# h-walk/PySlice

Measured on AMD Instinct MI355X. Metric: slice-steps/sec (probes x frames x slices / s), potential + slice loop + exit FFT, higher is better.
Workload: dtype complex64 (f32); 1 GPU; 64-probe STEM grid, 1024x1024 grid, 200 slices, 54 MD frames per GPU (BASELINE configs[2] per-frame work), 106583 atoms, 30 mrad, 100 keV; grid=1024, slices=200, probes=64, parallelism=frames x1, world_size_checked=1, frame_slots=59, frame_batch=4

## Files before the change

pyslice_amd/build_native.py:

```python
from __future__ import annotations

import os
import shutil
import subprocess
import sys

HERE = os.path.dirname(os.path.abspath(__file__))
CSRC = os.path.join(HERE, "csrc")
OUT = os.path.join(HERE, "libmslice.so")
SOURCES = ["mslice.hip", "slice_pass.hip", "slice_mixed_a.hip", "slice_mixed_b.hip", "slice_mixed_c.hip", "slice_mixed_d.hip", "slice_mixed_e.hip", "slice_mixed_f.hip", "tacaw_direct.hip", "tacaw_split.hip", "tacaw_split2.hip", "tacaw_welch.hip"]
def _deps():
    return sorted(f for f in os.listdir(CSRC) if f.endswith((".hip", ".h"))) + [os.path.join("..", "..", "include", "mslice.h")]
ARCH = "gfx950"


def _hipcc():
    for cand in (os.environ.get("HIPCC"), shutil.which("hipcc"), "/opt/rocm/bin/hipcc"):
        if cand and os.path.exists(cand):
            return cand
    raise RuntimeError("hipcc not found (ROCm toolchain required to build libmslice.so)")


def needs_build() -> bool:
    if not os.path.exists(OUT):
        return True
    t = os.path.getmtime(OUT)
    for d in _deps():
        p = os.path.join(CSRC, d)
        if os.path.exists(p) and os.path.getmtime(p) > t:
            return True
    return False


def build(force: bool = False, verbose: bool = True) -> str:
    if not force and not needs_build():
        return OUT
    from concurrent.futures import ThreadPoolExecutor
    objdir = os.path.join(HERE, "build")
    os.makedirs(objdir, exist_ok=True)
    flags = [f"--offload-arch={ARCH}", "-O3", "-std=c++17", "-fno-slp-vectorize", "-fPIC"]

    def compile_one(src):
        obj = os.path.join(objdir, os.path.splitext(src)[0] + ".o")
        cmd = [_hipcc()] + flags + ["-c", "-o", obj, src]
        if verbose:
            print("[pyslice_amd] " + " ".join(cmd), flush=True)
        subprocess.run(cmd, cwd=CSRC, check=True)
        return obj

    with ThreadPoolExecutor(max_workers=min(len(SOURCES), os.cpu_count() or 1)) as pool:
        objs = list(pool.map(compile_one, SOURCES))
    cmd = [_hipcc(), f"--offload-arch={ARCH}", "-shared", "-fPIC", "-o", OUT] + objs
    if verbose:
        print("[pyslice_amd] " + " ".join(cmd), flush=True)
    subprocess.run(cmd, cwd=CSRC, check=True)
    return OUT


if __name__ == "__main__":
    build(force="--force" in sys.argv)
    print(OUT)
```

pyslice_amd/csrc/mslice.hip:

```cpp
#include <hip/hip_runtime.h>

#include <algorithm>
#include <cmath>
#include <cstdarg>
#include <cstdio>
#include <cstdlib>
#include <cstring>
#include <string>
#include <type_traits>
#include <vector>

#include "../../include/mslice.h"
#include "fft_generic.h"
#include "fft_pow2.h"
#include "pot_ifft.h"
#include "rowtm_pass.h"
#include "potential.h"
#include "absorptive.h"
#include "finite.h"
#include "tds.h"
#include "ionization.h"
#include "slice_sums.h"
#include "thermal.h"
#include "phonons.h"
// ... 968 lines not shown
    case AX_TWO:
        job.tw = o.tw; job.tw2 = o.tw2; job.pl = o.ptab;
        return paired_dispatch(job, [&](auto in_p, auto out_p) { return launch_rowT2_io<decltype(in_p)::value, decltype(out_p)::value>(h, job, kind); });
    case AX_FOURSTEP:
        job.tw = (&o == &h->opx) ? h->tw4_x : h->tw4_y;
        return o.R == 32 ? launch_rowT_r<32>(h, job, kind) : launch_rowT_r<16>(h, job, kind);
    default:
        return fail(h, MSL_ERR_STATE, "transposing pass: the axis has no one-pass kernel");
    }
}

int slice_loop_onepass_b(msl_handle* h, int fused_slot, int groups, int first_group) {
    const msl_config& c = h->cfg;
    const int P = c.n_probes * groups, nz = c.nz;
    const size_t toff = (size_t)first_group * c.nz * c.nx * c.ny;
    const size_t npix = (size_t)c.nx * c.ny;
    const long long isA = (long long)c.nx * h->pitch, isB = (long long)c.ny * h->pitchT;
    const bool fused = fused_slot >= 0;
    int rc;
    if ((rc = begin_timed(h, nz + 4 + (fused ? tap_launches(h) : 0)))) return rc;
    for (int k = 0; k < nz; ++k) {
        RowTJob j{};
        j.flags = (k > 0 ? P2_PRE_A : 0) | (k < nz - 1 ? P2_POST_A : 0);
        if (h->debug_flags_mask >= 0) j.flags &= h->debug_flags_mask;
        j.n_images = P;
        set_frame_groups(h, j, groups);
        if (h->opx.kind == AX_WAVE2K && h->opy.kind == AX_WAVE2K)
            j.flags |= (k > 0 ? P2_IN_PAIRED : 0) | (k < nz - 1 ? P2_OUT_PAIRED : 0);
        if (interleaves(h->opx) && interleaves(h->opy) && !dbg_env("MSL_NO_INTERLEAVE") && h->debug_flags_mask < 0) {
            j.flags |= (k > 0 ? P2_IN_PAIRED : 0) | (k < nz - 1 ? P2_OUT_PAIRED : 0);
            j.perm_shift = (((k & 1) ? h->opy : h->opx).R == 32) ? 2 : 1;
        }
        if (!(k & 1)) {
            j.in = (k == 0) ? h->psi0 : h->psi; j.out = h->psiT;
            j.trans = h->trans + toff + (size_t)k * npix; j.pl = h->pyt;
            j.in_image_stride = isA; j.out_image_stride = isB; j.in_pitch = h->pitch; j.out_pitch = h->pitchT; j.n_lines = c.nx;
            rc = launch_rowT_dir(h, h->opy, j, K_ROW);
        } else {
            j.in = h->psiT; j.out = h->psi;
            j.trans = h->transT + toff + (size_t)k * npix; j.pl = h->pxt;
            j.in_image_stride = isB; j.out_image_stride = isA; j.in_pitch = h->pitchT; j.out_pitch = h->pitch; j.n_lines = c.ny;
            rc = launch_rowT_dir(h, h->opx, j, K_COL);
        }
        if (rc) return rc;
        if (k < nz - 1) {
            int rp = 0;
            const int order = tap_order((k & 1) ? h->opx : h->opy, j.flags, j.perm_shift, &rp);
            if ((rc = tap_step(h, k, fused_slot, groups, (k & 1) ? h->psi : h->psiT, !(k & 1), order, rp, (k & 1) ? 1 : 0))) return rc;
        }
    }
    if (nz & 1) {
        dim3 grid((c.nx + 31) / 32, (c.ny + 31) / 32, P);
        hipLaunchKernelGGL(transpose_kernel, grid, dim3(256), 0, h->stream, h->psiT, h->psi, c.ny, c.nx, h->pitchT, h->pitch, isB, isA);
        HIPCHK(h, hipGetLastError());
        if ((rc = mark_launch(h, K_OTHER))) return rc;
    }
    if (fused) {
        if (h->Ry) {
            RowJob r = row_job(h, h->psi, P, h->pitch);
            r.do_fft = true;
            if ((rc = launch_row_fast(h, r, K_OTHER))) return rc;
        } else {
            LineArgs r = row_args(h, h->psi, h->psi, P, h->pitch);
            r.fft1 = +1;
            if ((rc = launch_lines(h, h->plan_y, r, K_OTHER))) return rc;
        }
        if ((rc = epilogue_x_pass(h, fused_slot, groups))) return rc;
    }
    count_slice_loop(h, P, groups, fused, 16);
    return MSL_OK;
}

template <int R>
int launch_row2_r(msl_handle* h, Row2Job job, int kind) {
    constexpr int N = R * R, G = 256 / R;
    const size_t lds = (size_t)N * 16 + (size_t)G * R * (R + 1) * 4;
    const int per_cu = std::max(1, std::min(2, (int)((size_t)h->lds_limit / lds)));
    const int grid = chunked_grid(h, job, job.nx / G, (long long)h->n_cus * per_cu);
    hipLaunchKernelGGL(row_pass2_kernel<R>, dim3(grid), dim3(256), lds, h->stream, job);
    HIPCHK(h, hipGetLastError());
    return mark_launch(h, kind);
}

int slice_loop_onepass(msl_handle* h, int fused_slot, int groups, int first_group) {
    if (h->scheme_b) return slice_loop_onepass_b(h, fused_slot, groups, first_group);
    const msl_config& c = h->cfg;
    const int P = c.n_probes * groups, nz = c.nz;
    const size_t toff = (size_t)first_group * c.nz * c.nx * c.ny;
    const size_t npix = (size_t)c.nx * c.ny;
    const long long isA = (long long)c.nx * h->pitch, isB = (long long)c.ny * h->pitchT;
    const bool fused = fused_slot >= 0;
    int rc;
    if (nz == 1)
        HIPCHK(h, hipMemcpyAsync(h->psi, h->psi0, (size_t)P * isA * sizeof(float2), hipMemcpyDeviceToDevice, h->stream));
    if ((rc = begin_timed(h, nz + 2 + (fused ? tap_launches(h) : 0)))) return rc;
    for (int k = 0; k < nz; ++k) {
        const bool last = (k == nz - 1);
        int flags = (k > 0 ? P2_PRE_A : 0) | (!last ? P2_POST_A : 0) | ((last && fused) ? P2_POST_F : 0);
        if (h->debug_flags_mask >= 0) flags &= h->debug_flags_mask;
        if (last) {
            Row2Job j{};
            j.psi = h->psi; j.trans = h->trans + toff + (size_t)k * npix; j.py = h->pyt; j.tw = h->tw4_y;
            j.image_stride = isA; j.pitch = h->pitch; j.nx = c.nx; j.n_images = P; j.flags = flags;
            set_frame_groups(h, j, groups);
            rc = h->Ry == 32 ? launch_row2_r<32>(h, j, K_ROW) : launch_row2_r<16>(h, j, K_ROW);
            if (rc) return rc;
            break;
        }
        const bool along_y = !slice_is_transposed(h, k);
        RowTJob j{};
        if (!dbg_env("MSL_NO_INTERLEAVE") && h->debug_flags_mask < 0) flags |= (k > 0 ? P2_IN_PAIRED : 0) | (k < nz - 2 ? P2_OUT_PAIRED : 0);
        j.flags = flags; j.n_images = P;
        j.perm_shift = ((along_y ? h->Rx : h->Ry) == 32) ? 2 : 1;
        set_frame_groups(h, j, groups);
        if (along_y) {
            j.in = (k == 0) ? h->psi0 : h->psi; j.out = h->psiT;
            j.trans = h->trans + toff + (size_t)k * npix; j.pl = h->pyt; j.tw = h->tw4_y;
            j.in_image_stride = isA; j.out_image_stride = isB; j.in_pitch = h->pitch; j.out_pitch = h->pitchT; j.n_lines = c.nx;
            rc = h->Ry == 32 ? launch_rowT_r<32>(h, j, K_ROW) : launch_rowT_r<16>(h, j, K_ROW);
        } else {
            j.in = (k == 0) ? h->psi0T : h->psiT; j.out = h->psi;
            j.trans = h->transT + toff + (size_t)k * npix; j.pl = h->pxt; j.tw = h->tw4_x;
            j.in_image_stride = isB; j.out_image_stride = isA; j.in_pitch = h->pitchT; j.out_pitch = h->pitch; j.n_lines = c.ny;
            rc = h->Rx == 32 ? launch_rowT_r<32>(h, j, K_COL) : launch_rowT_r<16>(h, j, K_COL);
        }
        if (rc) return rc;
        const int order = (j.flags & P2_OUT_PAIRED) ? TAP_INTERLEAVED : TAP_NATURAL;
        if ((rc = tap_step(h, k, fused_slot, groups, along_y ? h->psiT : h->psi, along_y, order, 8 << j.perm_shift, along_y ? 0 : 1))) return rc;
    }
    if (fused && (rc = epilogue_x_pass(h, fused_slot, groups))) return rc;
    count_slice_loop(h, P, groups, fused, 16);
    return MSL_OK;
}

int ensure_atoms(msl_handle* h, size_t n, size_t rows) {
    int rc;
    if (rows <= h->atom_cap) return (h->fin_R > 0 && h->d_wgt.n < h->atom_cap) ? h->d_wgt.alloc(h, h->atom_cap) : MSL_OK;
    (void)n;
    size_t cap = std::max<size_t>(rows, h->atom_cap * 3 / 2 + 1024);
    if (h->fin_R > 0 && (rc = h->d_wgt.alloc(h, cap))) return rc;
    if ((rc = h->d_pos.alloc(h, cap * 3)) || (rc = h->d_Z.alloc(h, cap)) || (rc = h->d_key.alloc(h, cap)) || (rc = h->d_order.alloc(h, cap)) ||
        (rc = h->d_u1.alloc(h, cap)) || (rc = h->d_u2.alloc(h, cap))) return rc;
    if ((rc = h->d_ex.alloc(h, cap * (size_t)(h->cfg.nx / 2 + 1))) || (rc = h->d_ey.alloc(h, cap * (size_t)(h->cfg.ny / 2 + 1)))) return rc;
    h->atom_cap = cap;
    return MSL_OK;
}

struct TdsSignal : TdsSums {
    static constexpr const char* name = "tds";
    static constexpr const char* setter = "msl_set_tds";
    static int slots(int n) { return n; }
    static int slab_slots(int n) { return n; }
    template <typename F> static void with_slots(int k, F&& f) { with_int<1, 2, 3, 4>(k, f); }
    static bool on(const msl_handle* h) { return h->tds_on; }
    static bool built(const msl_handle* h) { return h->tds_W && h->abs_built; }
    static int n(const msl_handle* h) { return h->tds_n; }
    static const float* weights(const msl_handle* h) { return h->tds_W; }
    static DevBuf<double>& slab(msl_handle* h) { return h->tds_part; }
};
struct IonSignal : IonSums {
    static constexpr const char* name = "ionization";
    static constexpr const char* setter = "msl_set_ionization";
    static int slots(int n) { return n <= 1 ? 1 : n <= 2 ? 2 : n <= 4 ? 4 : 8; }
    static int slab_slots(int) { return ION_MAX; }
    template <typename F> static void with_slots(int k, F&& f) { with_int<1, 2, 4, 8>(k, f); }
    static bool on(const msl_handle* h) { return h->ion_on; }
    static bool built(const msl_handle* h) { return h->ion_W && h->ion_built; }
    static int n(const msl_handle* h) { return h->ion_n; }
    static const float* weights(const msl_handle* h) { return h->ion_W; }
    static DevBuf<float>& slab(msl_handle* h) { return h->ion_part; }
};

template <class S>
int slice_sums_queue(msl_handle* h, const float2* psi, int P, const float* w, size_t w_cs, int n, double* dst, int reps = 1) {
    const msl_config& c = h->cfg;
    const long long pairs = (long long)c.nx * ((c.ny + 1) / 2), n_tiles = (pairs + S::TILE - 1) / S::TILE;
    if (n_tiles > 0x7fffffffLL) return fail(h, MSL_ERR_UNSUPPORTED, "%s: too many tiles", S::name);
    const int slots = S::slots(n);
    auto& part = S::slab(h);
    int rc = part.reserve(h, (size_t)n_tiles * P * S::slab_slots(n));
    if (rc) return rc;
    const long long wg_slots = (long long)h->n_cus * 8;
    int pc = P;
    while (pc > 1 && n_tiles * ((P + pc - 1) / pc) < wg_slots) pc = (pc + 1) / 2;
    while ((P + pc - 1) / pc > 65535) ++pc;
    const bool vec = (h->pitch % 2 == 0) && (((uintptr_t)psi & 15) == 0);
    const dim3 grid((unsigned)n_tiles, (unsigned)((P + pc - 1) / pc));
    for (int r = 0; r < reps; ++r) {
        S::with_slots(slots, [&](auto k) { with_bool(vec, [&](auto v) {
            hipLaunchKernelGGL((slice_sums_kernel<typename S::kernel_policy, decltype(k)::value, decltype(v)::value>), grid, dim3(256), 0, h->stream,
                               psi, w, (long long)w_cs, n, c.nx, c.ny, h->pitch, P, pc, part.p);
        }); });
        HIPCHK(h, hipGetLastError());
        if (reps == 1 && (rc = mark_launch(h, K_OTHER))) return rc;
    }
    S::with_slots(slots, [&](auto k) {
        hipLaunchKernelGGL((slice_sums_finish_kernel<typename S::acc_t, decltype(k)::value>), dim3((unsigned)(((long long)P * slots + 255) / 256)),
                           dim3(256), 0, h->stream, part.p, n_tiles, P, n, dst);
    });
    HIPCHK(h, hipGetLastError());
    return reps == 1 ? mark_launch(h, K_OTHER) : MSL_OK;
}

template <class S>
int slice_sums_of_slice(msl_handle* h, const float2* psi, int P, int z, double* dst, int reps = 1) {
    const size_t npix = (size_t)h->cfg.nx * h->cfg.ny;
    return slice_sums_queue<S>(h, psi, P, S::weights(h) + (size_t)z * npix, npix * h->cfg.nz, S::n(h), dst, reps);
}
int slice_sums_hook(msl_handle* h, int P, int z) {
    return h->tds_on ? slice_sums_of_slice<TdsSignal>(h, h->psi, P, z, h->tds_acc + (size_t)z * P * h->tds_n)
                     : slice_sums_of_slice<IonSignal>(h, h->psi, P, z, h->ion_acc + (size_t)z * P * h->ion_n);
}

// ... 3506 lines not shown
```

pyslice_amd/csrc/rowt_pass.h:

```cpp
#pragma once
#include <type_traits>
#include <utility>
#include <hip/hip_runtime.h>
#include "fft_regs.h"
#include "kernel_util.h"
#include "rowt_frame.h"

#ifndef MSL_TW_LDS
#define MSL_TW_LDS 0
#endif
#ifndef MSL_DIT_LCH
#define MSL_DIT_LCH 8
#endif
#ifndef MSL_DIT_FENCE
#define MSL_DIT_FENCE 0
#endif
#ifndef MSL_STAGGER
#define MSL_STAGGER 4
#endif
#define MSL_IC(x) std::integral_constant<int, (x)>{}

namespace msl {


template <int R>
__device__ __forceinline__ void exchange_addtid(float2 (&v)[R], const float* scratch_base, unsigned wave_scratch, int ln, int lane64) {
    static_assert(64 % R == 0 && R % 4 == 0, "R-lane groups inside one wave; rows are read four floats at a time");
    constexpr int PW = 68;
    if constexpr (MSL_ABL2 & 4) return;
    const float* rd = scratch_base + ln * PW + (lane64 / R) * R;
    asm volatile("s_mov_b32 m0, %0\n\ts_nop 1" :: "s"(wave_scratch) : "memory");
#pragma unroll
    for (int k1 = 0; k1 < R; ++k1) asm volatile("ds_write_addtid_b32 %0 offset:%1" :: "v"(v[k1].x), "n"(k1 * PW * 4) : "memory");
    wave_lds_fence();
#pragma unroll
    for (int g = 0; g < R / 4; ++g) {
        const float4 q = *reinterpret_cast<const float4*>(rd + 4 * g);
        v[4 * g].x = q.x; v[4 * g + 1].x = q.y; v[4 * g + 2].x = q.z; v[4 * g + 3].x = q.w;
    }
    wave_lds_fence();
    asm volatile("s_mov_b32 m0, %0\n\ts_nop 1" :: "s"(wave_scratch) : "memory");
#pragma unroll
    for (int k1 = 0; k1 < R; ++k1) asm volatile("ds_write_addtid_b32 %0 offset:%1" :: "v"(v[k1].y), "n"(k1 * PW * 4) : "memory");
    wave_lds_fence();
#pragma unroll
    for (int g = 0; g < R / 4; ++g) {
        const float4 q = *reinterpret_cast<const float4*>(rd + 4 * g);
        v[4 * g].y = q.x; v[4 * g + 1].y = q.y; v[4 * g + 2].y = q.z; v[4 * g + 3].y = q.w;
    }
    wave_lds_fence();
}

template <int R, bool INV, int WMODE, int STRIDE, int C0, typename TabPtr, int... J>
__device__ __forceinline__ void dit_leaf_chunk(const float2* in, float2* v, TabPtr tab, int ln, std::integer_sequence<int, J...>) {
    constexpr int LR = dit_leaf_radix(R), C = R / LR;
    float2 w[sizeof...(J)][4];
    if constexpr (MSL_ABL2 & 16) {
        ((w[J][0] = tab[ln], w[J][1] = tab[ln], w[J][2] = tab[ln], w[J][3] = tab[ln]), ...);
    } else {
        ((w[J][0] = tab[(C0 + J) * STRIDE + ln], w[J][1] = tab[(C0 + J + C) * STRIDE + ln]), ...);
        if constexpr (LR == 4) ((w[J][2] = tab[(C0 + J + 2 * C) * STRIDE + ln], w[J][3] = tab[(C0 + J + 3 * C) * STRIDE + ln]), ...);
    }
    (dit_leaf<R, INV, WMODE, C0 + J>(in, v, w[J]), ...);
    (pin(v[C0 + J]), ...); (pin(v[C0 + J + C]), ...);
    if constexpr (LR == 4) { (pin(v[C0 + J + 2 * C]), ...); (pin(v[C0 + J + 3 * C]), ...); }
    __builtin_amdgcn_sched_barrier(0);
}
template <int R, bool INV, int WMODE, int STRIDE, int CH, int C0, typename TabPtr>
__device__ __forceinline__ void dit_leaf_chunks(const float2* in, float2* v, TabPtr tab, int ln) {
    if constexpr (C0 < dit_leaf_count(R)) {
        dit_leaf_chunk<R, INV, WMODE, STRIDE, C0>(in, v, tab, ln, std::make_integer_sequence<int, CH>{});
        dit_leaf_chunks<R, INV, WMODE, STRIDE, CH, C0 + CH>(in, v, tab, ln);
    }
}

template <int R, bool INV, int WMODE, int K, int I>
__device__ __forceinline__ void dit_leaves_regs_part(const float2* in, float2* v, const float2* w) {
    if constexpr (I < K) {
        constexpr int LR = dit_leaf_radix(R);
        float2 ww[4];
        ww[0] = w[I]; ww[1] = w[I + K];
        if constexpr (LR == 4) { ww[2] = w[I + 2 * K]; ww[3] = w[I + 3 * K]; }
        dit_leaf<R, INV, WMODE, I>(in, v, ww);
        dit_leaves_regs_part<R, INV, WMODE, K, I + 1>(in, v, w);
    }
}
constexpr int rowT_tw_reg_leaves(int R, int FL) { return (!MSL_TW_LDS && R == 32 && FL >= 0) ? 8 : 0; }
constexpr int ROWT_TW_REG_LCH = 4;

constexpr int rowT_cs(int R) { return (R * R + 33) / 32 * 32 + 2; }
template <int R, int LINES, bool IN_P, bool OUT_P, int FL>
__global__ void __launch_bounds__(LINES * R, (R == 16) ? 3 : 2) rowT_pass_kernel(RowTJob job) {
    constexpr int N = R * R;
    constexpr int NT = LINES * R;
    constexpr int CS = rowT_cs(R);
    constexpr int TWK = rowT_tw_reg_leaves(R, FL), LRW = dit_leaf_radix(R);
    constexpr bool TWR = TWK > 0;
    constexpr int LCH0 = TWR ? ROWT_TW_REG_LCH : MSL_DIT_LCH;
    constexpr int LCHL = LCH0 < dit_leaf_count(R) ? LCH0 : dit_leaf_count(R);
    constexpr int FN = MSL_DIT_FENCE;
    static_assert(LINES == 16, "16 lines = 128-byte transposed segments (8 lines / 64 bytes measured 1.6x slower)");
    static_assert(dit_leaf_count(R) % LCHL == 0 && TWK % LCHL == 0 && TWK < dit_leaf_count(R), "whole chunks");
    extern __shared__ __attribute__((aligned(16))) char smem_raw[];
    float2* tw = reinterpret_cast<float2*>(smem_raw);
    float2* pl = tw + N;
    float2* tile = pl + N;
    const int tid = threadIdx.x;
    for (int i = tid; i < N; i += NT) { tw[i] = job.tw[i]; pl[i] = job.pl[i]; }
    __syncthreads();
    const int grp = tid / R, ln = tid % R;
    float2 twr[TWR ? LRW * TWK : 1];
    if constexpr (TWR) {
#pragma unroll
        for (int i = 0; i < LRW * TWK; ++i) twr[i] = tw[((i % TWK) + (i / TWK) * dit_leaf_count(R)) * R + ln];
        pin_all(twr);
    }
    const int l64 = tid & 63;
    float2* myrow = tile + grp * CS;
    const float* wscr = reinterpret_cast<const float*>(tile + (grp - grp % (64 / R)) * CS);
    const unsigned wscr_lds = __builtin_amdgcn_readfirstlane((unsigned)(size_t)(tile + (grp - grp % (64 / R)) * CS));
    const bool pre_a = (MSL_ABL2 & 8) ? false : FL >= 0 ? (FL & P2_PRE_A) != 0 : (job.flags & P2_PRE_A) != 0;
    const bool post_a = (MSL_ABL2 & 8) ? false : FL >= 0 ? (FL & P2_POST_A) != 0 : (job.flags & P2_POST_A) != 0;
    auto line_of = [&](int lbb) {
        if constexpr (OUT_P) {
            const int sh = job.perm_shift;
            return (((lbb >> sh) * 2 + (grp & 1)) << (sh + 3)) + 8 * (lbb & ((1 << sh) - 1)) + (grp >> 1);
        } else {
            return lbb * LINES + grp;
        }
    };
    auto line_ptr = [&](const RowTCursor& c) {
        return job.in + (long long)c.image() * job.in_image_stride + (long long)line_of(c.lb) * job.in_pitch;
    };
    auto load_regs = [&](float2 (&dst)[R], const float2* r, auto lo_c, auto hi_c) {
        constexpr int LO = decltype(lo_c)::value, HI = decltype(hi_c)::value;
        if constexpr (IN_P) {
            static_assert(LO % 2 == 0 && HI % 2 == 0, "register pairs");
#pragma unroll
            for (int jp = LO / 2; jp < HI / 2; ++jp) {
                const msl_f4v t = __builtin_nontemporal_load(reinterpret_cast<const msl_f4v*>(r + (2 * R * jp + 2 * ln)));
                dst[2 * jp] = make_float2(t.x, t.y); dst[2 * jp + 1] = make_float2(t.z, t.w);
            }
        } else {
#pragma unroll
            for (int j = LO; j < HI; ++j) dst[j] = ld_stream(r + (j * R + ln));
        }
    };
    RowTCursor cur = RowTCursor::first(job, job.n_lines / LINES);
    float2 vn[R];
    if (cur.valid()) load_regs(vn, line_ptr(cur), MSL_IC(0), MSL_IC(R));
    __builtin_amdgcn_s_waitcnt(0x0F70);
    float2 tv[R];
#ifdef MSL_CLOCK
    const unsigned long long clk0 = __builtin_amdgcn_s_memtime(), rt0 = __builtin_amdgcn_s_memrealtime();
#endif
    while (cur.valid()) {
        if constexpr (MSL_STAGGER > 0)
            for (int i = __builtin_amdgcn_readfirstlane(tid >> 6) & 3; i > 0; --i) __builtin_amdgcn_s_sleep(MSL_STAGGER);
        float2 v[R];
        if (cur.k == 0) {
            const float2* trow = rowt_trans_row(job, cur, line_of(cur.lb), N);
#pragma unroll
            for (int j = 0; j < R; ++j) tv[j] = ld_stream(trow + j * R + ln);
        }
        const RowTCursor nxt = cur.next();
        const float2* nptr = line_ptr(cur.prefetch_target(nxt));
        auto pfx = [&](auto i_c) {
            constexpr int I = decltype(i_c)::value;
            constexpr int LO = (R * I / 16) & ~1, HI = (R * (I + 1) / 16) & ~1;
            if constexpr (HI > LO && !(MSL_ABL2 & 1)) {
                __builtin_amdgcn_sched_barrier(0);
                load_regs(vn, nptr, MSL_IC(LO), MSL_IC(HI));
                __builtin_amdgcn_sched_barrier(0);
            }
        };
#define MSL_HALF_TAB(INV, WM, TAB, I0) do { dit_leaf_chunks<R, INV, WM, R, LCHL, 0>(v, v, TAB, ln); pfx(MSL_IC(I0)); \
                                            dit_upper<R, INV, FN>(v); pin_all(v); pfx(MSL_IC((I0) + 1)); } while (0)
#define MSL_HALF_TW(INV, WM, I0) do { \
            if constexpr (TWR) { dit_leaves_regs_part<R, INV, WM, TWK, 0>(v, v, twr); \
                                 dit_leaf_chunks<R, INV, WM, R, LCHL, TWK>(v, v, tw, ln); pin_all(v); pfx(MSL_IC(I0)); \
                                 dit_upper<R, INV, FN>(v); pin_all(v); pfx(MSL_IC((I0) + 1)); } \
            else MSL_HALF_TAB(INV, WM, tw, I0); } while (0)
        if (pre_a) {
            dit_leaves_plain<R, false, 0>(vn, v); pin_all(v);
            pfx(MSL_IC(0));
            dit_upper<R, false, FN>(v); pin_all(v);
            pfx(MSL_IC(1));
            exchange_addtid<R>(v, wscr, wscr_lds, ln, l64);
            MSL_HALF_TW(false, 1, 2);
            MSL_HALF_TAB(true, 1, pl, 4);
            exchange_addtid<R>(v, wscr, wscr_lds, ln, l64);
            MSL_HALF_TW(true, 2, 6);
        } else {
#pragma unroll
            for (int j = 0; j < R; ++j) v[j] = vn[j];
            pin_all(v);
            pfx(MSL_IC(0)); pfx(MSL_IC(1)); pfx(MSL_IC(2)); pfx(MSL_IC(3)); pfx(MSL_IC(4)); pfx(MSL_IC(5)); pfx(MSL_IC(6)); pfx(MSL_IC(7));
        }
        if (post_a) {
            dit_leaves_regs<R, false, 1, 0>(v, v, tv); pin_all(v);
            pfx(MSL_IC(8));
            dit_upper<R, false, FN>(v); pin_all(v);
            pfx(MSL_IC(9));
            exchange_addtid<R>(v, wscr, wscr_lds, ln, l64);
            MSL_HALF_TW(false, 1, 10);
            MSL_HALF_TAB(true, 1, pl, 12);
            exchange_addtid<R>(v, wscr, wscr_lds, ln, l64);
            MSL_HALF_TW(true, 2, 14);
        } else {
#pragma unroll
            for (int j = 0; j < R; ++j) v[j] = cmulf(v[j], tv[j]);
            pfx(MSL_IC(8)); pfx(MSL_IC(9)); pfx(MSL_IC(10)); pfx(MSL_IC(11)); pfx(MSL_IC(12)); pfx(MSL_IC(13)); pfx(MSL_IC(14)); pfx(MSL_IC(15));
        }
#undef MSL_HALF_TW
#undef MSL_HALF_TAB
        if constexpr (MSL_ABL2 & 32) {
            float acc = 0.f;
#pragma unroll
            for (int j = 0; j < R; ++j) acc += v[j].x + v[j].y;
            if (acc == 1.2345e-30f) job.out[tid] = make_float2(acc, acc);
        } else {
            wave_lds_fence();
#pragma unroll
            for (int j = 0; j < R; ++j) myrow[j * R + ln] = v[j];
            lds_barrier();
            tile_store_transposed<LINES, NT, CS, N, false, true>(tile, rowt_out_image(job, cur) + cur.lb * LINES, job.out_pitch, N, tid);
            lds_barrier();
        }
        cur = nxt;
    }
#ifdef MSL_CLOCK
    if (tid == 0 && job.clk) {
        job.clk[2 * blockIdx.x] = __builtin_amdgcn_s_memtime() - clk0;
        job.clk[2 * blockIdx.x + 1] = __builtin_amdgcn_s_memrealtime() - rt0;
    }
#endif
}

constexpr size_t rowT_lds_bytes(int R) { return ((size_t)2 * R * R + (size_t)16 * rowT_cs(R)) * 8; }

bool rowT_launch(int R, const RowTJob& job, int grid, size_t lds_limit, hipStream_t stream);
int rowT_selftest(hipStream_t stream);

}
```

pyslice_amd/csrc/slice_pass.hip:

```cpp
#include "rowt_pass.h"

namespace msl {

template <int R, bool IN_P, bool OUT_P, int FL>
static bool launch_one(const RowTJob& job, int grid, size_t lds_limit, hipStream_t stream) {
    (void)hipFuncSetAttribute((const void*)rowT_pass_kernel<R, 16, IN_P, OUT_P, FL>, hipFuncAttributeMaxDynamicSharedMemorySize, (int)lds_limit);
    hipLaunchKernelGGL((rowT_pass_kernel<R, 16, IN_P, OUT_P, FL>), dim3(grid), dim3(16 * R), rowT_lds_bytes(R), stream, job);
    return true;
}

template <int R>
static bool launch_r(const RowTJob& job, int grid, size_t lds_limit, hipStream_t stream) {
    const bool in_p = job.flags & P2_IN_PAIRED, out_p = job.flags & P2_OUT_PAIRED;
    const int fl = job.flags & (P2_PRE_A | P2_POST_A);
    if (in_p && out_p && fl == 3) return launch_one<R, true, true, 3>(job, grid, lds_limit, stream);
    if (!in_p && out_p && fl == 2) return launch_one<R, false, true, 2>(job, grid, lds_limit, stream);
    if (in_p && !out_p && fl == 1) return launch_one<R, true, false, 1>(job, grid, lds_limit, stream);
    if (in_p && !out_p && fl == 3) return launch_one<R, true, false, 3>(job, grid, lds_limit, stream);
    if (!in_p && !out_p && fl == 3) return launch_one<R, false, false, 3>(job, grid, lds_limit, stream);
    if (!in_p && !out_p) return launch_one<R, false, false, -1>(job, grid, lds_limit, stream);
    return false;
}

bool rowT_launch(int R, const RowTJob& job, int grid, size_t lds_limit, hipStream_t stream) {
    if (R == 32) return launch_r<32>(job, grid, lds_limit, stream);
    if (R == 16) return launch_r<16>(job, grid, lds_limit, stream);
    return false;
}

template <int R>
__global__ void __launch_bounds__(64) exchange_selftest_kernel(int* bad) {
    __shared__ __attribute__((aligned(16))) float scr[R * 68];
    const int lane = threadIdx.x, g = lane / R, l = lane % R;
    float2 v[R];
#pragma unroll
    for (int j = 0; j < R; ++j) v[j] = make_float2((float)(1000 * g + 32 * j + l), -(float)(1000 * g + 32 * j + l));
    const unsigned base = __builtin_amdgcn_readfirstlane((unsigned)(size_t)scr);
    exchange_addtid<R>(v, scr, base, l, lane);
    int wrong = 0;
#pragma unroll
    for (int j = 0; j < R; ++j) {
        const float want = (float)(1000 * g + 32 * l + j);
        wrong += (v[j].x != want) + (v[j].y != -want);
    }
    if (wrong) atomicAdd(bad, wrong);
}

int rowT_selftest(hipStream_t stream) {
    int* bad = nullptr;
    if (hipMalloc(&bad, sizeof(int)) != hipSuccess) return -1;
    int host = -1;
    bool ok = hipMemsetAsync(bad, 0, sizeof(int), stream) == hipSuccess;
    if (ok) {
        hipLaunchKernelGGL(exchange_selftest_kernel<32>, dim3(1), dim3(64), 0, stream, bad);
        hipLaunchKernelGGL(exchange_selftest_kernel<16>, dim3(1), dim3(64), 0, stream, bad);
        ok = hipGetLastError() == hipSuccess && hipMemcpyAsync(&host, bad, sizeof(int), hipMemcpyDeviceToHost, stream) == hipSuccess &&
             hipStreamSynchronize(stream) == hipSuccess;
    }
    (void)hipFree(bad);
    return ok ? host : -1;
}

}
```

Baseline: 230,300 slice-steps/s.

## Replace last-slice row2 and epilogue with transposing exit-tail passes

For the final slice, the Row2 kernel plus separate epilogue x-pass is replaced by two transposing passes. The first applies the last slice's propagation, transmission and forward y-FFT and writes to the transposed buffer. The second performs the forward x-FFT with an fftshift-style rotation, storing directly into the fused output slot with probe/frame remapping. The intent is to remove redundant full-grid passes and the inverse half of the final propagation, at the cost of new kernel variants and an extra code path gated by many conditions.

```diff
diff --git a/pyslice_amd/build_native.py b/pyslice_amd/build_native.py
--- a/pyslice_amd/build_native.py
+++ b/pyslice_amd/build_native.py
@@ -8,7 +8,7 @@
 HERE = os.path.dirname(os.path.abspath(__file__))
 CSRC = os.path.join(HERE, "csrc")
 OUT = os.path.join(HERE, "libmslice.so")
-SOURCES = ["mslice.hip", "slice_pass.hip", "slice_mixed_a.hip", "slice_mixed_b.hip", "slice_mixed_c.hip", "slice_mixed_d.hip", "slice_mixed_e.hip", "slice_mixed_f.hip", "tacaw_direct.hip", "tacaw_split.hip", "tacaw_split2.hip", "tacaw_welch.hip"]
+SOURCES = ["mslice.hip", "slice_pass.hip", "slice_exit.hip", "slice_mixed_a.hip", "slice_mixed_b.hip", "slice_mixed_c.hip", "slice_mixed_d.hip", "slice_mixed_e.hip", "slice_mixed_f.hip", "tacaw_direct.hip", "tacaw_split.hip", "tacaw_split2.hip", "tacaw_welch.hip"]
 def _deps():
     return sorted(f for f in os.listdir(CSRC) if f.endswith((".hip", ".h"))) + [os.path.join("..", "..", "include", "mslice.h")]
 ARCH = "gfx950"
diff --git a/pyslice_amd/csrc/mslice.hip b/pyslice_amd/csrc/mslice.hip
--- a/pyslice_amd/csrc/mslice.hip
+++ b/pyslice_amd/csrc/mslice.hip
@@ -1074,6 +1074,38 @@
     return mark_launch(h, kind);
 }
 
+bool exit_tail_transposes(const msl_handle* h, int fused_slot) {
+    const msl_config& c = h->cfg;
+    return fused_slot >= 0 && h->onepass && !h->scheme_b && h->opx.kind == AX_FOURSTEP && h->opy.kind == AX_FOURSTEP && c.ny % 32 == 0 &&
+           h->wx == c.nx && h->wy == c.ny && h->bin_stage == nullptr &&!h->tds_on && !h->ion_on && h->debug_flags_mask < 0 && !dbg_env("MSL_OLD_EXIT_TAIL");
+}
+
+int exit_tail_passes(msl_handle* h, int slot, int groups, size_t toff) {
+    const msl_config& c = h->cfg;
+    const int P = c.n_probes * groups, nz = c.nz;
+    const size_t npix = (size_t)c.nx * c.ny;
+    int rc;
+    RowTJob j{};
+    j.flags = (nz > 1 ? P2_PRE_A : 0) | P2_POST_F; j.n_images = P;
+    set_frame_groups(h, j, groups);
+    j.in = (nz == 1) ? h->psi0 : h->psi; j.out = h->psiT;
+    j.trans = h->trans + toff + (size_t)(nz - 1) * npix; j.pl = h->pyt; j.tw = h->tw4_y;
+    j.in_image_stride = (long long)c.nx * h->pitch; j.out_image_stride = (long long)c.ny * h->pitchT;
+    j.in_pitch = h->pitch; j.out_pitch = h->pitchT; j.n_lines = c.nx;
+    if ((rc = h->Ry == 32 ? launch_rowT_r<32>(h, j, K_ROW) : launch_rowT_r<16>(h, j, K_ROW))) return rc;
+    RowTJob x{};
+    x.in = h->psiT; x.out = h->wf + (size_t)slot * h->wpitch; x.tw = h->tw4_x;
+    x.in_image_stride = j.out_image_stride; x.in_pitch = h->pitchT; x.n_lines = c.ny; x.n_images = P; x.pchunk = 1;
+    x.out_pitch = h->wy; x.out_image_stride = (long long)c.n_frames * h->wpitch;
+    if (groups > 1) { x.t_group = c.n_probes; x.t_magic = (unsigned)((1ull << 32) / (unsigned)c.n_probes + 1); x.t_stride = (long long)h->wpitch; }
+    const size_t lds = rowT_exit_lds_bytes(h->Rx);
+    const int per_cu = std::max(1, std::min(h->Rx == 16 ? 3 : 2, (int)((size_t)h->lds_limit / lds)));
+    const int grid = (int)std::min<long long>((long long)(c.ny / 16) * P, (long long)h->n_cus * per_cu);
+    if (!rowT_exit_launch(h->Rx, x, grid, (size_t)h->lds_limit, h->stream)) return fail(h, MSL_ERR_STATE, "exit pass: no kernel for %d points", c.nx);
+    HIPCHK(h, hipGetLastError());
+    return mark_launch(h, K_OTHER);
+}
+
 int slice_loop_onepass(msl_handle* h, int fused_slot, int groups, int first_group) {
     if (h->scheme_b) return slice_loop_onepass_b(h, fused_slot, groups, first_group);
     const msl_config& c = h->cfg;
@@ -1082,14 +1114,19 @@
     const size_t npix = (size_t)c.nx * c.ny;
     const long long isA = (long long)c.nx * h->pitch, isB = (long long)c.ny * h->pitchT;
     const bool fused = fused_slot >= 0;
+    const bool xtail = exit_tail_transposes(h, fused_slot);
     int rc;
-    if (nz == 1)
+    if (nz == 1 && !xtail)
         HIPCHK(h, hipMemcpyAsync(h->psi, h->psi0, (size_t)P * isA * sizeof(float2), hipMemcpyDeviceToDevice, h->stream));
     if ((rc = begin_timed(h, nz + 2 + (fused ? tap_launches(h) : 0)))) return rc;
     for (int k = 0; k < nz; ++k) {
         const bool last = (k == nz - 1);
         int flags = (k > 0 ? P2_PRE_A : 0) | (!last ? P2_POST_A : 0) | ((last && fused) ? P2_POST_F : 0);
         if (h->debug_flags_mask >= 0) flags &= h->debug_flags_mask;
+        if (last && xtail) {
+            if ((rc = exit_tail_passes(h, fused_slot, groups, toff))) return rc;
+            break;
+        }
         if (last) {
             Row2Job j{};
             j.psi = h->psi; j.trans = h->trans + toff + (size_t)k * npix; j.py = h->pyt; j.tw = h->tw4_y;
@@ -1120,7 +1157,7 @@
         const int order = (j.flags & P2_OUT_PAIRED) ? TAP_INTERLEAVED : TAP_NATURAL;
         if ((rc = tap_step(h, k, fused_slot, groups, along_y ? h->psiT : h->psi, along_y, order, 8 << j.perm_shift, along_y ? 0 : 1))) return rc;
     }
-    if (fused && (rc = epilogue_x_pass(h, fused_slot, groups))) return rc;
+    if (fused && !xtail && (rc = epilogue_x_pass(h, fused_slot, groups))) return rc;
     count_slice_loop(h, P, groups, fused, 16);
     return MSL_OK;
 }
diff --git a/pyslice_amd/csrc/rowt_pass.h b/pyslice_amd/csrc/rowt_pass.h
--- a/pyslice_amd/csrc/rowt_pass.h
+++ b/pyslice_amd/csrc/rowt_pass.h
@@ -91,155 +91,83 @@
 constexpr int rowT_cs(int R) { return (R * R + 33) / 32 * 32 + 2; }
 template <int R, int LINES, bool IN_P, bool OUT_P, int FL>
 __global__ void __launch_bounds__(LINES * R, (R == 16) ? 3 : 2) rowT_pass_kernel(RowTJob job) {
-    constexpr int N = R * R;
-    constexpr int NT = LINES * R;
-    constexpr int CS = rowT_cs(R);
-    constexpr int TWK = rowT_tw_reg_leaves(R, FL), LRW = dit_leaf_radix(R);
-    constexpr bool TWR = TWK > 0;
-    constexpr int LCH0 = TWR ? ROWT_TW_REG_LCH : MSL_DIT_LCH;
-    constexpr int LCHL = LCH0 < dit_leaf_count(R) ? LCH0 : dit_leaf_count(R);
-    constexpr int FN = MSL_DIT_FENCE;
-    static_assert(LINES == 16, "16 lines = 128-byte transposed segments (8 lines / 64 bytes measured 1.6x slower)");
-    static_assert(dit_leaf_count(R) % LCHL == 0 && TWK % LCHL == 0 && TWK < dit_leaf_count(R), "whole chunks");
+#include "rowt_pass_body.h"
+}
+
+template <int R, int LINES, bool PRE>
+__global__ void __launch_bounds__(LINES * R, (R == 16) ? 3 : 2) rowT_last_kernel(RowTJob job) {
+    constexpr bool IN_P = false, OUT_P = false;
+    constexpr int FL = (PRE ? P2_PRE_A : 0) | P2_POST_F;
+#include "rowt_pass_body.h"
+}
+
+constexpr int ROWT_EXIT_LCH = 8;
+template <int R, int LINES>
+__global__ void __launch_bounds__(LINES * R, (R == 16) ? 3 : 2) rowT_exit_kernel(RowTJob job) {
+    constexpr int N = R * R, NT = LINES * R, CS = rowT_cs(R);
+    constexpr int LCHL = ROWT_EXIT_LCH < dit_leaf_count(R) ? ROWT_EXIT_LCH : dit_leaf_count(R);
+    static_assert(LINES == 16 && dit_leaf_count(R) % LCHL == 0 && R % 8 == 0, "128-byte segments, whole chunks, whole quarters");
     extern __shared__ __attribute__((aligned(16))) char smem_raw[];
     float2* tw = reinterpret_cast<float2*>(smem_raw);
-    float2* pl = tw + N;
-    float2* tile = pl + N;
+    float2* tile = tw + N;
     const int tid = threadIdx.x;
-    for (int i = tid; i < N; i += NT) { tw[i] = job.tw[i]; pl[i] = job.pl[i]; }
+    for (int i = tid; i < N; i += NT) tw[i] = job.tw[i];
     __syncthreads();
-    const int grp = tid / R, ln = tid % R;
-    float2 twr[TWR ? LRW * TWK : 1];
-    if constexpr (TWR) {
-#pragma unroll
-        for (int i = 0; i < LRW * TWK; ++i) twr[i] = tw[((i % TWK) + (i / TWK) * dit_leaf_count(R)) * R + ln];
-        pin_all(twr);
-    }
-    const int l64 = tid & 63;
+    const int grp = tid / R, ln = tid % R, l64 = tid & 63;
     float2* myrow = tile + grp * CS;
     const float* wscr = reinterpret_cast<const float*>(tile + (grp - grp % (64 / R)) * CS);
     const unsigned wscr_lds = __builtin_amdgcn_readfirstlane((unsigned)(size_t)(tile + (grp - grp % (64 / R)) * CS));
-    const bool pre_a = (MSL_ABL2 & 8) ? false : FL >= 0 ? (FL & P2_PRE_A) != 0 : (job.flags & P2_PRE_A) != 0;
-    const bool post_a = (MSL_ABL2 & 8) ? false : FL >= 0 ? (FL & P2_POST_A) != 0 : (job.flags & P2_POST_A) != 0;
-    auto line_of = [&](int lbb) {
-        if constexpr (OUT_P) {
-            const int sh = job.perm_shift;
-            return (((lbb >> sh) * 2 + (grp & 1)) << (sh + 3)) + 8 * (lbb & ((1 << sh) - 1)) + (grp >> 1);
-        } else {
-            return lbb * LINES + grp;
-        }
-    };
     auto line_ptr = [&](const RowTCursor& c) {
-        return job.in + (long long)c.image() * job.in_image_stride + (long long)line_of(c.lb) * job.in_pitch;
-    };
-    auto load_regs = [&](float2 (&dst)[R], const float2* r, auto lo_c, auto hi_c) {
-        constexpr int LO = decltype(lo_c)::value, HI = decltype(hi_c)::value;
-        if constexpr (IN_P) {
-            static_assert(LO % 2 == 0 && HI % 2 == 0, "register pairs");
-#pragma unroll
-            for (int jp = LO / 2; jp < HI / 2; ++jp) {
-                const msl_f4v t = __builtin_nontemporal_load(reinterpret_cast<const msl_f4v*>(r + (2 * R * jp + 2 * ln)));
-                dst[2 * jp] = make_float2(t.x, t.y); dst[2 * jp + 1] = make_float2(t.z, t.w);
-            }
-        } else {
-#pragma unroll
-            for (int j = LO; j < HI; ++j) dst[j] = ld_stream(r + (j * R + ln));
-        }
+        return job.in + (long long)c.image() * job.in_image_stride + (long long)(c.lb * LINES + grp) * job.in_pitch;
     };
     RowTCursor cur = RowTCursor::first(job, job.n_lines / LINES);
     float2 vn[R];
-    if (cur.valid()) load_regs(vn, line_ptr(cur), MSL_IC(0), MSL_IC(R));
-    __builtin_amdgcn_s_waitcnt(0x0F70);
-    float2 tv[R];
-#ifdef MSL_CLOCK
-    const unsigned long long clk0 = __builtin_amdgcn_s_memtime(), rt0 = __builtin_amdgcn_s_memrealtime();
-#endif
+    if (cur.valid()) {
+        const float2* r = line_ptr(cur);
+#pragma unroll
+        for (int j = 0; j < R; ++j) vn[j] = ld_stream(r + (j * R + ln));
+    }
     while (cur.valid()) {
-        if constexpr (MSL_STAGGER > 0)
-            for (int i = __builtin_amdgcn_readfirstlane(tid >> 6) & 3; i > 0; --i) __builtin_amdgcn_s_sleep(MSL_STAGGER);
-        float2 v[R];
-        if (cur.k == 0) {
-            const float2* trow = rowt_trans_row(job, cur, line_of(cur.lb), N);
-#pragma unroll
-            for (int j = 0; j < R; ++j) tv[j] = ld_stream(trow + j * R + ln);
-        }
         const RowTCursor nxt = cur.next();
         const float2* nptr = line_ptr(cur.prefetch_target(nxt));
         auto pfx = [&](auto i_c) {
             constexpr int I = decltype(i_c)::value;
-            constexpr int LO = (R * I / 16) & ~1, HI = (R * (I + 1) / 16) & ~1;
-            if constexpr (HI > LO && !(MSL_ABL2 & 1)) {
-                __builtin_amdgcn_sched_barrier(0);
-                load_regs(vn, nptr, MSL_IC(LO), MSL_IC(HI));
-                __builtin_amdgcn_sched_barrier(0);
-            }
+            __builtin_amdgcn_sched_barrier(0);
+#pragma unroll
+            for (int j = R * I / 4; j < R * (I + 1) / 4; ++j) vn[j] = ld_stream(nptr + (j * R + ln));
+            __builtin_amdgcn_sched_barrier(0);
         };
-#define MSL_HALF_TAB(INV, WM, TAB, I0) do { dit_leaf_chunks<R, INV, WM, R, LCHL, 0>(v, v, TAB, ln); pfx(MSL_IC(I0)); \
-                                            dit_upper<R, INV, FN>(v); pin_all(v); pfx(MSL_IC((I0) + 1)); } while (0)
-#define MSL_HALF_TW(INV, WM, I0) do { \
-            if constexpr (TWR) { dit_leaves_regs_part<R, INV, WM, TWK, 0>(v, v, twr); \
-                                 dit_leaf_chunks<R, INV, WM, R, LCHL, TWK>(v, v, tw, ln); pin_all(v); pfx(MSL_IC(I0)); \
-                                 dit_upper<R, INV, FN>(v); pin_all(v); pfx(MSL_IC((I0) + 1)); } \
-            else MSL_HALF_TAB(INV, WM, tw, I0); } while (0)
-        if (pre_a) {
-            dit_leaves_plain<R, false, 0>(vn, v); pin_all(v);
-            pfx(MSL_IC(0));
-            dit_upper<R, false, FN>(v); pin_all(v);
-            pfx(MSL_IC(1));
-            exchange_addtid<R>(v, wscr, wscr_lds, ln, l64);
-            MSL_HALF_TW(false, 1, 2);
-            MSL_HALF_TAB(true, 1, pl, 4);
-            exchange_addtid<R>(v, wscr, wscr_lds, ln, l64);
-            MSL_HALF_TW(true, 2, 6);
-        } else {
+        float2 v[R];
+        dit_leaves_plain<R, false, 0>(vn, v); pin_all(v);
+        pfx(MSL_IC(0));
+        dit_upper<R, false, 0>(v); pin_all(v);
+        pfx(MSL_IC(1));
+        exchange_addtid<R>(v, wscr, wscr_lds, ln, l64);
+        dit_leaf_chunks<R, false, 1, R, LCHL, 0>(v, v, tw, ln); pin_all(v);
+        pfx(MSL_IC(2));
+        dit_upper<R, false, 0>(v); pin_all(v);
+        pfx(MSL_IC(3));
+        wave_lds_fence();
 #pragma unroll
-            for (int j = 0; j < R; ++j) v[j] = vn[j];
-            pin_all(v);
-            pfx(MSL_IC(0)); pfx(MSL_IC(1)); pfx(MSL_IC(2)); pfx(MSL_IC(3)); pfx(MSL_IC(4)); pfx(MSL_IC(5)); pfx(MSL_IC(6)); pfx(MSL_IC(7));
-        }
-        if (post_a) {
-            dit_leaves_regs<R, false, 1, 0>(v, v, tv); pin_all(v);
-            pfx(MSL_IC(8));
-            dit_upper<R, false, FN>(v); pin_all(v);
-            pfx(MSL_IC(9));
-            exchange_addtid<R>(v, wscr, wscr_lds, ln, l64);
-            MSL_HALF_TW(false, 1, 10);
-            MSL_HALF_TAB(true, 1, pl, 12);
-            exchange_addtid<R>(v, wscr, wscr_lds, ln, l64);
-            MSL_HALF_TW(true, 2, 14);
-        } else {
-#pragma unroll
-            for (int j = 0; j < R; ++j) v[j] = cmulf(v[j], tv[j]);
-            pfx(MSL_IC(8)); pfx(MSL_IC(9)); pfx(MSL_IC(10)); pfx(MSL_IC(11)); pfx(MSL_IC(12)); pfx(MSL_IC(13)); pfx(MSL_IC(14)); pfx(MSL_IC(15));
-        }
-#undef MSL_HALF_TW
-#undef MSL_HALF_TAB
-        if constexpr (MSL_ABL2 & 32) {
-            float acc = 0.f;
-#pragma unroll
-            for (int j = 0; j < R; ++j) acc += v[j].x + v[j].y;
-            if (acc == 1.2345e-30f) job.out[tid] = make_float2(acc, acc);
-        } else {
-            wave_lds_fence();
-#pragma unroll
-            for (int j = 0; j < R; ++j) myrow[j * R + ln] = v[j];
-            lds_barrier();
-            tile_store_transposed<LINES, NT, CS, N, false, true>(tile, rowt_out_image(job, cur) + cur.lb * LINES, job.out_pitch, N, tid);
-            lds_barrier();
-        }
+        for (int j = 0; j < R; ++j) myrow[((j + R / 2) % R) * R + ln] = v[j];
+        lds_barrier();
+        const unsigned p = (unsigned)__builtin_amdgcn_readfirstlane(cur.image());
+        const unsigned f = job.t_group <= 0 ? 0u : job.t_group == 1 ? p : __umulhi(p, job.t_magic);
+        const unsigned probe = job.t_group <= 0 ? p : p - f * (unsigned)job.t_group;
+        int c0 = cur.lb * LINES + job.n_lines / 2;
+        if (c0 >= job.n_lines) c0 -= job.n_lines;
+        float2* dst = job.out + (long long)probe * job.out_image_stride + (long long)f * job.t_stride + c0;
+        tile_store_transposed<LINES, NT, CS, N, false, true>(tile, dst, job.out_pitch, N, tid);
+        lds_barrier();
         cur = nxt;
     }
-#ifdef MSL_CLOCK
-    if (tid == 0 && job.clk) {
-        job.clk[2 * blockIdx.x] = __builtin_amdgcn_s_memtime() - clk0;
-        job.clk[2 * blockIdx.x + 1] = __builtin_amdgcn_s_memrealtime() - rt0;
-    }
-#endif
 }
 
 constexpr size_t rowT_lds_bytes(int R) { return ((size_t)2 * R * R + (size_t)16 * rowT_cs(R)) * 8; }
+constexpr size_t rowT_exit_lds_bytes(int R) { return ((size_t)R * R + (size_t)16 * rowT_cs(R)) * 8; }
 
 bool rowT_launch(int R, const RowTJob& job, int grid, size_t lds_limit, hipStream_t stream);
+bool rowT_exit_launch(int R, const RowTJob& job, int grid, size_t lds_limit, hipStream_t stream);
 int rowT_selftest(hipStream_t stream);
 
 }
diff --git a/pyslice_amd/csrc/rowt_pass_body.h b/pyslice_amd/csrc/rowt_pass_body.h
--- /dev/null
+++ b/pyslice_amd/csrc/rowt_pass_body.h
@@ -0,0 +1,154 @@
+    constexpr int N = R * R;
+    constexpr int NT = LINES * R;
+    constexpr int CS = rowT_cs(R);
+    constexpr int TWK = rowT_tw_reg_leaves(R, FL), LRW = dit_leaf_radix(R);
+    constexpr bool TWR = TWK > 0;
+    constexpr int LCH0 = TWR ? ROWT_TW_REG_LCH : MSL_DIT_LCH;
+    constexpr int LCHL = LCH0 < dit_leaf_count(R) ? LCH0 : dit_leaf_count(R);
+    constexpr int FN = MSL_DIT_FENCE;
+    constexpr bool POST_F = FL >= 0 && (FL & P2_POST_F) != 0;
+    static_assert(!POST_F || (!(FL & P2_POST_A) && !OUT_P), "the forward-only ending replaces the second half and writes natural order");
+    static_assert(LINES == 16, "16 lines = 128-byte transposed segments (8 lines / 64 bytes measured 1.6x slower)");
+    static_assert(dit_leaf_count(R) % LCHL == 0 && TWK % LCHL == 0 && TWK < dit_leaf_count(R), "whole chunks");
+    extern __shared__ __attribute__((aligned(16))) char smem_raw[];
+    float2* tw = reinterpret_cast<float2*>(smem_raw);
+    float2* pl = tw + N;
+    float2* tile = pl + N;
+    const int tid = threadIdx.x;
+    for (int i = tid; i < N; i += NT) { tw[i] = job.tw[i]; pl[i] = job.pl[i]; }
+    __syncthreads();
+    const int grp = tid / R, ln = tid % R;
+    float2 twr[TWR ? LRW * TWK : 1];
+    if constexpr (TWR) {
+#pragma unroll
+        for (int i = 0; i < LRW * TWK; ++i) twr[i] = tw[((i % TWK) + (i / TWK) * dit_leaf_count(R)) * R + ln];
+        pin_all(twr);
+    }
+    const int l64 = tid & 63;
+    float2* myrow = tile + grp * CS;
+    const float* wscr = reinterpret_cast<const float*>(tile + (grp - grp % (64 / R)) * CS);
+    const unsigned wscr_lds = __builtin_amdgcn_readfirstlane((unsigned)(size_t)(tile + (grp - grp % (64 / R)) * CS));
+    const bool pre_a = (MSL_ABL2 & 8) ? false : FL >= 0 ? (FL & P2_PRE_A) != 0 : (job.flags & P2_PRE_A) != 0;
+    const bool post_a = (MSL_ABL2 & 8) ? false : FL >= 0 ? (FL & P2_POST_A) != 0 : (job.flags & P2_POST_A) != 0;
+    auto line_of = [&](int lbb) {
+        if constexpr (OUT_P) {
+            const int sh = job.perm_shift;
+            return (((lbb >> sh) * 2 + (grp & 1)) << (sh + 3)) + 8 * (lbb & ((1 << sh) - 1)) + (grp >> 1);
+        } else {
+            return lbb * LINES + grp;
+        }
+    };
+    auto line_ptr = [&](const RowTCursor& c) {
+        return job.in + (long long)c.image() * job.in_image_stride + (long long)line_of(c.lb) * job.in_pitch;
+    };
+    auto load_regs = [&](float2 (&dst)[R], const float2* r, auto lo_c, auto hi_c) {
+        constexpr int LO = decltype(lo_c)::value, HI = decltype(hi_c)::value;
+        if constexpr (IN_P) {
+            static_assert(LO % 2 == 0 && HI % 2 == 0, "register pairs");
+#pragma unroll
+            for (int jp = LO / 2; jp < HI / 2; ++jp) {
+                const msl_f4v t = __builtin_nontemporal_load(reinterpret_cast<const msl_f4v*>(r + (2 * R * jp + 2 * ln)));
+                dst[2 * jp] = make_float2(t.x, t.y); dst[2 * jp + 1] = make_float2(t.z, t.w);
+            }
+        } else {
+#pragma unroll
+            for (int j = LO; j < HI; ++j) dst[j] = ld_stream(r + (j * R + ln));
+        }
+    };
+    RowTCursor cur = RowTCursor::first(job, job.n_lines / LINES);
+    float2 vn[R];
+    if (cur.valid()) load_regs(vn, line_ptr(cur), MSL_IC(0), MSL_IC(R));
+    __builtin_amdgcn_s_waitcnt(0x0F70);
+    float2 tv[R];
+#ifdef MSL_CLOCK
+    const unsigned long long clk0 = __builtin_amdgcn_s_memtime(), rt0 = __builtin_amdgcn_s_memrealtime();
+#endif
+    while (cur.valid()) {
+        if constexpr (MSL_STAGGER > 0)
+            for (int i = __builtin_amdgcn_readfirstlane(tid >> 6) & 3; i > 0; --i) __builtin_amdgcn_s_sleep(MSL_STAGGER);
+        float2 v[R];
+        if (cur.k == 0) {
+            const float2* trow = rowt_trans_row(job, cur, line_of(cur.lb), N);
+#pragma unroll
+            for (int j = 0; j < R; ++j) tv[j] = ld_stream(trow + j * R + ln);
+        }
+        const RowTCursor nxt = cur.next();
+        const float2* nptr = line_ptr(cur.prefetch_target(nxt));
+        auto pfx = [&](auto i_c) {
+            constexpr int I = decltype(i_c)::value;
+            constexpr int LO = (R * I / 16) & ~1, HI = (R * (I + 1) / 16) & ~1;
+            if constexpr (HI > LO && !(MSL_ABL2 & 1)) {
+                __builtin_amdgcn_sched_barrier(0);
+                load_regs(vn, nptr, MSL_IC(LO), MSL_IC(HI));
+                __builtin_amdgcn_sched_barrier(0);
+            }
+        };
+#define MSL_HALF_TAB(INV, WM, TAB, I0) do { dit_leaf_chunks<R, INV, WM, R, LCHL, 0>(v, v, TAB, ln); pfx(MSL_IC(I0)); \
+                                            dit_upper<R, INV, FN>(v); pin_all(v); pfx(MSL_IC((I0) + 1)); } while (0)
+#define MSL_HALF_TW(INV, WM, I0) do { \
+            if constexpr (TWR) { dit_leaves_regs_part<R, INV, WM, TWK, 0>(v, v, twr); \
+                                 dit_leaf_chunks<R, INV, WM, R, LCHL, TWK>(v, v, tw, ln); pin_all(v); pfx(MSL_IC(I0)); \
+                                 dit_upper<R, INV, FN>(v); pin_all(v); pfx(MSL_IC((I0) + 1)); } \
+            else MSL_HALF_TAB(INV, WM, tw, I0); } while (0)
+        if (pre_a) {
+            dit_leaves_plain<R, false, 0>(vn, v); pin_all(v);
+            pfx(MSL_IC(0));
+            dit_upper<R, false, FN>(v); pin_all(v);
+            pfx(MSL_IC(1));
+            exchange_addtid<R>(v, wscr, wscr_lds, ln, l64);
+            MSL_HALF_TW(false, 1, 2);
+            MSL_HALF_TAB(true, 1, pl, 4);
+            exchange_addtid<R>(v, wscr, wscr_lds, ln, l64);
+            MSL_HALF_TW(true, 2, 6);
+        } else {
+#pragma unroll
+            for (int j = 0; j < R; ++j) v[j] = vn[j];
+            pin_all(v);
+            pfx(MSL_IC(0)); pfx(MSL_IC(1)); pfx(MSL_IC(2)); pfx(MSL_IC(3)); pfx(MSL_IC(4)); pfx(MSL_IC(5)); pfx(MSL_IC(6)); pfx(MSL_IC(7));
+        }
+        if constexpr (POST_F) {
+            dit_leaves_regs<R, false, 1, 0>(v, v, tv); pin_all(v);
+            pfx(MSL_IC(8));
+            dit_upper<R, false, FN>(v); pin_all(v);
+            pfx(MSL_IC(9));
+            exchange_addtid<R>(v, wscr, wscr_lds, ln, l64);
+            MSL_HALF_TW(false, 1, 10);
+            pfx(MSL_IC(12)); pfx(MSL_IC(13)); pfx(MSL_IC(14)); pfx(MSL_IC(15));
+        } else if (post_a) {
+            dit_leaves_regs<R, false, 1, 0>(v, v, tv); pin_all(v);
+            pfx(MSL_IC(8));
+            dit_upper<R, false, FN>(v); pin_all(v);
+            pfx(MSL_IC(9));
+            exchange_addtid<R>(v, wscr, wscr_lds, ln, l64);
+            MSL_HALF_TW(false, 1, 10);
+            MSL_HALF_TAB(true, 1, pl, 12);
+            exchange_addtid<R>(v, wscr, wscr_lds, ln, l64);
+            MSL_HALF_TW(true, 2, 14);
+        } else {
+#pragma unroll
+            for (int j = 0; j < R; ++j) v[j] = cmulf(v[j], tv[j]);
+            pfx(MSL_IC(8)); pfx(MSL_IC(9)); pfx(MSL_IC(10)); pfx(MSL_IC(11)); pfx(MSL_IC(12)); pfx(MSL_IC(13)); pfx(MSL_IC(14)); pfx(MSL_IC(15));
+        }
+#undef MSL_HALF_TW
+#undef MSL_HALF_TAB
+        if constexpr (MSL_ABL2 & 32) {
+            float acc = 0.f;
+#pragma unroll
+            for (int j = 0; j < R; ++j) acc += v[j].x + v[j].y;
+            if (acc == 1.2345e-30f) job.out[tid] = make_float2(acc, acc);
+        } else {
+            wave_lds_fence();
+#pragma unroll
+            for (int j = 0; j < R; ++j) myrow[j * R + ln] = v[j];
+            lds_barrier();
+            tile_store_transposed<LINES, NT, CS, N, false, true>(tile, rowt_out_image(job, cur) + cur.lb * LINES, job.out_pitch, N, tid);
+            lds_barrier();
+        }
+        cur = nxt;
+    }
+#ifdef MSL_CLOCK
+    if (tid == 0 && job.clk) {
+        job.clk[2 * blockIdx.x] = __builtin_amdgcn_s_memtime() - clk0;
+        job.clk[2 * blockIdx.x + 1] = __builtin_amdgcn_s_memrealtime() - rt0;
+    }
+#endif
diff --git a/pyslice_amd/csrc/slice_exit.hip b/pyslice_amd/csrc/slice_exit.hip
--- /dev/null
+++ b/pyslice_amd/csrc/slice_exit.hip
@@ -0,0 +1,18 @@
+#include "rowt_pass.h"
+
+namespace msl {
+
+template <int R>
+static bool launch_exit(const RowTJob& job, int grid, size_t lds_limit, hipStream_t stream) {
+    (void)hipFuncSetAttribute((const void*)rowT_exit_kernel<R, 16>, hipFuncAttributeMaxDynamicSharedMemorySize, (int)lds_limit);
+    hipLaunchKernelGGL((rowT_exit_kernel<R, 16>), dim3(grid), dim3(16 * R), rowT_exit_lds_bytes(R), stream, job);
+    return true;
+}
+
+bool rowT_exit_launch(int R, const RowTJob& job, int grid, size_t lds_limit, hipStream_t stream) {
+    if (R == 32) return launch_exit<32>(job, grid, lds_limit, stream);
+    if (R == 16) return launch_exit<16>(job, grid, lds_limit, stream);
+    return false;
+}
+
+}
diff --git a/pyslice_amd/csrc/slice_pass.hip b/pyslice_amd/csrc/slice_pass.hip
--- a/pyslice_amd/csrc/slice_pass.hip
+++ b/pyslice_amd/csrc/slice_pass.hip
@@ -9,10 +9,21 @@
     return true;
 }
 
+template <int R, bool PRE>
+static bool launch_last(const RowTJob& job, int grid, size_t lds_limit, hipStream_t stream) {
+    (void)hipFuncSetAttribute((const void*)rowT_last_kernel<R, 16, PRE>, hipFuncAttributeMaxDynamicSharedMemorySize, (int)lds_limit);
+    hipLaunchKernelGGL((rowT_last_kernel<R, 16, PRE>), dim3(grid), dim3(16 * R), rowT_lds_bytes(R), stream, job);
+    return true;
+}
+
 template <int R>
 static bool launch_r(const RowTJob& job, int grid, size_t lds_limit, hipStream_t stream) {
     const bool in_p = job.flags & P2_IN_PAIRED, out_p = job.flags & P2_OUT_PAIRED;
     const int fl = job.flags & (P2_PRE_A | P2_POST_A);
+    if (job.flags & P2_POST_F) {
+        if (in_p || out_p || (fl & P2_POST_A)) return false;
+        return fl ? launch_last<R, true>(job, grid, lds_limit, stream) : launch_last<R, false>(job, grid, lds_limit, stream);
+    }
     if (in_p && out_p && fl == 3) return launch_one<R, true, true, 3>(job, grid, lds_limit, stream);
     if (!in_p && out_p && fl == 2) return launch_one<R, false, true, 2>(job, grid, lds_limit, stream);
     if (in_p && !out_p && fl == 1) return launch_one<R, true, false, 1>(job, grid, lds_limit, stream);
```

New measurement: 230,800 slice-steps/s, median of 6. About the same (+0.2%).
